# openjamoses/TOSEM-2021-Replication

Hardware: NVIDIA H100
Metric: source MB/s scanned (tokenise + line-hash + classify + aggregate) (higher is better)
Workload: dtype u8

## Files before the change

### tosem-2021-replication_b200/csrc/tsm_api.cu

```cuda
#include <algorithm>
#include <cstdio>
#include <cstdlib>
#include <cstring>
#include <new>
#include <vector>

#include "tsm_device.cuh"

#include "tsm_scan_kernels.cuh"
#include "tsm_scan_walk.cuh"
#include "tsm_reduce_kernels.cuh"
#include "tsm_diff_kernels.cuh"
#include "tsm_blame_kernels.cuh"
#include "tsm_stmt_kernels.cuh"
#include "tsm_lines_kernels.cuh"
#include "tsm_similar_kernels.cuh"

using namespace tsm;

static const char* const kNames[TSM_K] = TSM_CAT_NAMES_INIT;

struct ScratchPool {
  struct Slot { void* p; size_t cap; bool used; };
  std::vector<Slot> slots;
// ... 328 lines not shown
  CU(cudaSetDevice(c->device));
  cudaStream_t st = (cudaStream_t)stream;
  CallOrder order(c, st);
  CU(order.wait());
  rc = upload_index(c, k, st);
  if (rc != TSM_OK) return rc;
  if (c->n_files) CU(cudaMemcpyAsync(c->d_arena, k->arena, (size_t)c->arena_bytes, cudaMemcpyHostToDevice, st));
  c->resident = true;
  c->scanned = false;
  return TSM_OK;
}

static int ensure_event_buffers(tsm_ctx* c, uint32_t flags) {
  if ((flags & TSM_SCAN_ASSERT_EVENTS) && !c->d_aev)
    CU(cudaMalloc((void**)&c->d_aev, sizeof(tsm_assert_event) * (size_t)c->max_events));
  if ((flags & TSM_SCAN_HEADER_EVENTS) && !c->d_hev)
    CU(cudaMalloc((void**)&c->d_hev, sizeof(tsm_header_event) * (size_t)c->max_events));
  return TSM_OK;
}

static ScanParams make_params(const tsm_ctx* c, uint32_t flags) {
  ScanParams p{};
  p.arena = c->d_arena; p.off = c->d_off; p.len = c->d_len; p.ext = c->d_ext; p.grp = c->d_grp;
  p.n_files = c->n_files; p.n_groups = c->n_groups;
  p.unit_file = c->d_unit_file; p.unit_begin = c->d_unit_begin; p.unit_cap = c->unit_cap;
  p.ctrl = c->d_ctrl; p.stats = c->d_stats;
  p.cand = c->d_cand; p.cand_cap = (uint32_t)c->max_events;
  p.hev = c->d_hev; p.hev_cap = (uint32_t)c->max_events;
  p.aev = c->d_aev; p.aev_cap = (uint32_t)c->max_events;
  p.counts = c->d_counts; p.flags = flags; p.four = 4; p.cls_last = 1;
  return p;
}

static int classify_per_sm(tsm_ctx* c, size_t smem) {
  if (c->cls_smem != smem) {
    int per_sm = 0;
    if (cudaOccupancyMaxActiveBlocksPerMultiprocessor(&per_sm, k_classify_t<false>, 256, smem) != cudaSuccess || per_sm < 1) per_sm = 4;
    c->cls_per_sm = per_sm;
    c->cls_smem = smem;
  }
  return c->cls_per_sm;
}

static int launch_scan(tsm_ctx* c, uint32_t flags, cudaStream_t st, const tsm_corpus* host, bool check_files_here = false) {
  int rc = ensure_event_buffers(c, flags);
  if (rc != TSM_OK) return rc;
  ScanParams p = make_params(c, flags);
  const int n = c->n_files;
  c->launches = 0;
  CU(cudaMemsetAsync(c->d_zero, 0, (size_t)(reinterpret_cast<uint8_t*>(c->d_counts) - c->d_zero) +
                     sizeof(unsigned long long) * ((size_t)(c->n_groups + 1) * TSM_K + 4), st));
  if (n) {
    std::vector<int32_t> cut{0};
    if (host) {
      int64_t slab_bytes = 32ll << 20;
      while (c->arena_bytes / slab_bytes + 1 > tsm_ctx::kMaxSlabs) slab_bytes *= 2;
      int64_t next = slab_bytes;
      for (int32_t i = 1; i < n; ++i)
        if ((int64_t)host->off[i] >= next) { cut.push_back(i); next = (int64_t)host->off[i] + slab_bytes; }
      CU(cudaEventRecord(c->ready_ev, st));
      CU(cudaStreamWaitEvent(c->copy_stream, c->ready_ev, 0));
    }
    cut.push_back(n);
    if ((int)cut.size() - 1 > tsm_ctx::kMaxSlabs) return TSM_E_LAYOUT;
    const int es = c->ev_next;
    c->ev_next = (es + 1) % tsm_ctx::kRing;
    fold_events(c, es);
    cudaEvent_t* ev = c->ev[es];
    CU(cudaEventRecord(ev[0], st));
    const int n_slabs = (int)cut.size() - 1;
    const size_t hist = CLS_SMEM_BASE + sizeof(uint32_t) * (c->n_groups <= 16 ? (size_t)c->n_groups * TSM_K : 0);
    const int cls_grid = c->sms * classify_per_sm(c, hist);
    for (int s = 0; s < n_slabs; ++s) {
      const int32_t f0 = cut[(size_t)s], f1 = cut[(size_t)s + 1];
      if (host) {
        if (check_files_here && s == 0) {
          const int rc0 = check_files(host, f0, f1, true, true);
          if (rc0 != TSM_OK) return rc0;
        }
        const size_t b0 = (size_t)host->off[f0], b1 = (size_t)host->off[f1];
        CU(cudaMemcpyAsync(c->d_arena + b0, host->arena + b0, b1 - b0, cudaMemcpyHostToDevice, c->copy_stream));
        CU(cudaEventRecord(c->slab_ev[s], c->copy_stream));
        CU(cudaStreamWaitEvent(st, c->slab_ev[s], 0));
        if (check_files_here && s + 1 < n_slabs) {
          const int rc1 = check_files(host, f1, cut[(size_t)s + 2], true, true);
          if (rc1 != TSM_OK) { cudaStreamSynchronize(c->copy_stream); cudaStreamSynchronize(st); return rc1; }
        }
      }
      p.slab = c->d_slab + s; p.f_begin = f0; p.f_end = f1;
      p.unit_base = (uint32_t)((host ? (int64_t)host->off[f0] : 0) / CH + f0);
      k_plan<<<(f1 - f0 + 255) / 256, 256, 0, st>>>(p);
      CU(cudaGetLastError());
      if (s == 0 && n_slabs == 1) CU(cudaEventRecord(ev[1], st));
      if (flags & TSM_SCAN_REV_B) k_scan_t<true><<<c->sms * SCAN2_CTAS_PER_SM, SCAN2_WARPS * 32, SCAN2_SMEM_B, st>>>(p);
      else k_scan_t<false><<<c->sms * SCAN2_CTAS_PER_SM, SCAN2_WARPS * 32, SCAN2_SMEM, st>>>(p);
      CU(cudaGetLastError());
      if (s + 1 < n_slabs) {
        p.cls_last = 0;
        if (flags & TSM_SCAN_REV_B) k_classify_t<true><<<cls_grid, 256, hist, st>>>(p);
        else k_classify_t<false><<<cls_grid, 256, hist, st>>>(p);
        CU(cudaGetLastError());
        p.cls_last = 1;
      }
    }
    if (n_slabs > 1) CU(cudaEventRecord(ev[1], st));
    CU(cudaEventRecord(ev[2], st));
    if (flags & TSM_SCAN_REV_B) k_classify_t<true><<<cls_grid, 256, hist, st>>>(p);
    else k_classify_t<false><<<cls_grid, 256, hist, st>>>(p);
    CU(cudaGetLastError());
    CU(cudaEventRecord(ev[3], st));
    CU(cudaEventRecord(ev[4], st));
    c->ev_used[es] = (n_slabs == 1);
    c->ev_last = es;
    c->launches = 3 * n_slabs;
    CU(cudaGetLastError());
  }
  c->last_flags = flags;
  c->scanned = true;
  return TSM_OK;
}

extern "C" int tsm_scan_resident(tsm_ctx* c, uint32_t flags, void* stream) {
  if (!c) return TSM_E_ARG;
  flags &= TSM_SCAN_ASSERT_EVENTS | TSM_SCAN_HEADER_EVENTS | TSM_SCAN_REV_B;
  if (!c->resident) return TSM_E_STATE;
  CU(cudaSetDevice(c->device));
  CallOrder order(c, (cudaStream_t)stream);
  CU(order.wait());
  return launch_scan(c, flags, (cudaStream_t)stream, nullptr);
}

extern "C" int tsm_device_counts(tsm_ctx* c, void** dptr, int64_t* n_int64) {
  if (!c || !dptr || !n_int64) return TSM_E_ARG;
  if (!c->scanned) return TSM_E_STATE;
  *dptr = c->d_counts;
  *n_int64 = (int64_t)(c->n_groups + 1) * TSM_K + 4;
  return TSM_OK;
}

extern "C" int tsm_last_launch_count(tsm_ctx* c) { return c ? c->launches : 0; }

#if TSM_PHASE_CLOCKS
extern "C" int tsm_phase_clocks(unsigned long long* out, int n, int reset) {
  if (!out || n < (int)PH_N) return TSM_E_ARG;
  CU(cudaDeviceSynchronize());
  CU(cudaMemcpyFromSymbol(out, g_scan_phase_clk, sizeof(unsigned long long) * PH_N));
  if (reset) {
    const unsigned long long zero[PH_N] = {};
    CU(cudaMemcpyToSymbol(g_scan_phase_clk, zero, sizeof(zero)));
  }
  return TSM_OK;
}
#endif

extern "C" int tsm_last_kernel_ms(tsm_ctx* c, float* ms4) {
  if (!c || !ms4) return TSM_E_ARG;
  if (!c->scanned || c->n_files == 0 || c->ev_last < 0) return TSM_E_STATE;
  CU(cudaSetDevice(c->device));
  cudaEvent_t* ev = c->ev[c->ev_last];
  CU(cudaEventSynchronize(ev[4]));
  for (int i = 0; i < 4; ++i) CU(cudaEventElapsedTime(&ms4[i], ev[i], ev[i + 1]));
  return TSM_OK;
}

extern "C" int tsm_kernel_ms_stats(tsm_ctx* c, double* sum_ms4, int64_t* n_scans, int reset) {
  if (!c) return TSM_E_ARG;
  CU(cudaSetDevice(c->device));
  for (int i = 0; i < tsm_ctx::kRing; ++i) fold_events(c, i);
  if (sum_ms4) for (int k = 0; k < 4; ++k) sum_ms4[k] = c->ms_sum[k];
  if (n_scans) *n_scans = c->ms_n;
  if (reset) { for (double& v : c->ms_sum) v = 0; c->ms_n = 0; }
  return TSM_OK;
}

static int grow_event_buffers(tsm_ctx* c, int64_t need) {
  if (need <= c->max_events) return TSM_OK;
  if (need > 0xFFFFFFF0ll) return TSM_E_CAPACITY;
  unsigned long long* cand = nullptr;
  tsm_assert_event* aev = nullptr;
  tsm_header_event* hev = nullptr;
  const bool ok = cudaMalloc((void**)&cand, sizeof(unsigned long long) * (size_t)need) == cudaSuccess &&
                  (!c->d_aev || cudaMalloc((void**)&aev, sizeof(tsm_assert_event) * (size_t)need) == cudaSuccess) &&
                  (!c->d_hev || cudaMalloc((void**)&hev, sizeof(tsm_header_event) * (size_t)need) == cudaSuccess);
  if (!ok) {
    cudaGetLastError();
    cudaFree(cand); cudaFree(aev); cudaFree(hev);
    return TSM_E_CUDA;
  }
  cudaFree(c->d_cand); cudaFree(c->d_aev); cudaFree(c->d_hev);
  c->d_cand = cand; c->d_aev = aev; c->d_hev = hev;
  c->max_events = need;
  return TSM_OK;
}

static int download_tables(tsm_ctx* c, tsm_result* r, cudaStream_t st) {
  const int n = c->n_files, G = c->n_groups;
  unsigned long long* h_tot = reinterpret_cast<unsigned long long*>(c->h_ctrl + 1);
  CU(cudaMemcpyAsync(c->h_ctrl, c->d_ctrl, sizeof(Ctrl), cudaMemcpyDeviceToHost, st));
  CU(cudaMemcpyAsync(h_tot, c->d_counts + (size_t)(G + 1) * TSM_K, 4 * sizeof(unsigned long long), cudaMemcpyDeviceToHost, st));
  if (r->stats && n) CU(cudaMemcpyAsync(r->stats, c->d_stats, sizeof(tsm_file_stat) * (size_t)n, cudaMemcpyDeviceToHost, st));
  if (r->group_counts) CU(cudaMemcpyAsync(r->group_counts, c->d_counts, sizeof(int64_t) * (size_t)G * TSM_K, cudaMemcpyDeviceToHost, st));
  if (r->global_counts) CU(cudaMemcpyAsync(r->global_counts, c->d_counts + (size_t)G * TSM_K, sizeof(int64_t) * TSM_K, cudaMemcpyDeviceToHost, st));
  CU(cudaStreamSynchronize(st));
  for (int i = 0; i < 4; ++i) r->totals[i] = (int64_t)h_tot[i];
  return TSM_OK;
}

template <typename Event> static void sort_events_by_file(Event* ev, uint32_t m, int32_t n_files) {
  if (m < 2) return;
  std::vector<uint32_t> pos((size_t)n_files + 1, 0);
  for (uint32_t i = 0; i < m; ++i) pos[(size_t)ev[i].file + 1]++;
  for (int32_t f = 0; f < n_files; ++f) pos[(size_t)f + 1] += pos[(size_t)f];
  std::vector<Event> tmp(m);
  std::vector<uint32_t> at(pos.begin(), pos.end() - 1);
  for (uint32_t i = 0; i < m; ++i) tmp[at[ev[i].file]++] = ev[i];
  for (int32_t f = 0; f < n_files; ++f)
    if (pos[(size_t)f + 1] - pos[(size_t)f] > 1)
      std::sort(tmp.begin() + pos[(size_t)f], tmp.begin() + pos[(size_t)f + 1],
                [](const Event& a, const Event& b) { return a.line_off < b.line_off; });
  std::copy(tmp.begin(), tmp.end(), ev);
}

static int download(tsm_ctx* c, tsm_result* r, cudaStream_t st) {
  r->n_aev = 0; r->n_hev = 0;
  int rc = download_tables(c, r, st);
  if (rc != TSM_OK) return rc;
  if (c->h_ctrl->overflow) {
    const Ctrl& k = *c->h_ctrl;
    rc = grow_event_buffers(c, std::max<int64_t>(k.n_cand, std::max(k.n_hev, k.n_aev)));
    if (rc == TSM_OK) rc = launch_scan(c, c->last_flags, st, nullptr);
    if (rc == TSM_OK) rc = download_tables(c, r, st);
    if (rc != TSM_OK) return rc;
    if (c->h_ctrl->overflow) return TSM_E_CAPACITY;
  }
  const bool want_aev = (c->last_flags & TSM_SCAN_ASSERT_EVENTS) && r->aev, want_hev = (c->last_flags & TSM_SCAN_HEADER_EVENTS) && r->hev;
  if ((want_aev && (int64_t)c->h_ctrl->n_aev > r->aev_cap) || (want_hev && (int64_t)c->h_ctrl->n_hev > r->hev_cap)) {
    r->n_aev = c->h_ctrl->n_aev; r->n_hev = c->h_ctrl->n_hev;
    return TSM_E_CAPACITY;
  }
  if (want_aev) {
    const uint32_t m = c->h_ctrl->n_aev;
    CU(cudaMemcpyAsync(r->aev, c->d_aev, sizeof(tsm_assert_event) * (size_t)m, cudaMemcpyDeviceToHost, st));
    CU(cudaStreamSynchronize(st));
    sort_events_by_file(r->aev, m, c->n_files);
    r->n_aev = m;
  } else if (c->last_flags & TSM_SCAN_ASSERT_EVENTS) r->n_aev = c->h_ctrl->n_aev;
  if (want_hev) {
    const uint32_t m = c->h_ctrl->n_hev;
    CU(cudaMemcpyAsync(r->hev, c->d_hev, sizeof(tsm_header_event) * (size_t)m, cudaMemcpyDeviceToHost, st));
    CU(cudaStreamSynchronize(st));
    sort_events_by_file(r->hev, m, c->n_files);
    r->n_hev = m;
  } else if (c->last_flags & TSM_SCAN_HEADER_EVENTS) r->n_hev = c->h_ctrl->n_hev;
  return TSM_OK;
}

extern "C" int tsm_download(tsm_ctx* c, tsm_result* r, void* stream) {
  if (!c || !r) return TSM_E_ARG;
  if (!c->scanned) return TSM_E_STATE;
  CU(cudaSetDevice(c->device));
  CallOrder order(c, (cudaStream_t)stream);
  CU(order.wait());
  return download(c, r, (cudaStream_t)stream);
}

extern "C" int tsm_scan(tsm_ctx* c, const tsm_corpus* k, tsm_result* r, uint32_t flags, void* stream) {
  if (!c || !r) return TSM_E_ARG;
  int rc = check_corpus_head(c, k);
  if (rc != TSM_OK) return rc;
  flags &= TSM_SCAN_ASSERT_EVENTS | TSM_SCAN_HEADER_EVENTS | TSM_SCAN_REV_B;
  CU(cudaSetDevice(c->device));
  cudaStream_t st = (cudaStream_t)stream;
  CallOrder order(c, st);
  CU(order.wait());
  rc = upload_index(c, k, st);
  if (rc != TSM_OK) return rc;
  c->resident = true;
  rc = launch_scan(c, flags, st, k, true);
  if (rc != TSM_OK) { c->resident = false; c->scanned = false; return rc; }
  return download(c, r, st);
}

extern "C" int tsm_reduce(tsm_ctx* c, const uint8_t* flags, const int32_t* repo, const int32_t* case_id,
                          int32_t n_rows, int32_t n_flags, int32_t n_repos, int32_t n_cases,
                          int64_t* out, int64_t* cases_per_repo, void* stream) {
  if (!c || n_rows < 0 || n_flags < 0 || n_repos <= 0 || n_cases <= 0 || !out || (n_rows && (!flags || !repo || !case_id)))
    return TSM_E_ARG;
  for (int32_t i = 0; i < n_rows; ++i)
    if (repo[i] < 0 || repo[i] >= n_repos || case_id[i] < 0 || case_id[i] >= n_cases) return TSM_E_ARG;
  CU(cudaSetDevice(c->device));
  PoolScope pool_scope(&c->pool);
  cudaStream_t st = (cudaStream_t)stream;
  CallOrder order(c, st);
  CU(order.wait());
  const size_t words = ((size_t)n_cases + 31) / 32;
  const size_t nbits = (size_t)(n_flags + 1) * n_repos * words;
  DevBuf b_flags, b_repo, b_case, b_bits, b_out;
  SyncGuard guard(st);
  if (!b_flags.alloc((size_t)n_rows * n_flags) || !b_repo.alloc(sizeof(int32_t) * (size_t)n_rows) ||
      !b_case.alloc(sizeof(int32_t) * (size_t)n_rows) || !b_bits.alloc(sizeof(uint32_t) * nbits) ||
      !b_out.alloc(sizeof(unsigned long long) * (size_t)(n_flags + 1) * n_repos))
    return TSM_E_CUDA;
  uint8_t* d_flags = b_flags.as<uint8_t>(); int32_t *d_repo = b_repo.as<int32_t>(), *d_case = b_case.as<int32_t>();
  uint32_t* d_bits = b_bits.as<uint32_t>();
  unsigned long long* d_out = b_out.as<unsigned long long>();
  int rc = TSM_OK;
// ... 868 lines not shown
```

### tosem-2021-replication_b200/csrc/tsm_scan_kernels.cuh

```cuda
#pragma once
#include "tsm_device.cuh"

namespace tsm {

__constant__ uint32_t c_lut[256];
__constant__ uint32_t c_lut_b[256];
__constant__ uint32_t c_elut[256];
__device__ uint8_t c_cat_slot[TSM_CAT_SLOTS];
__device__ uint16_t c_cat_off[TSM_CAT_NAMED + 1];
__device__ char c_cat_blob[TSM_CAT_BLOB_LEN + 1];

__global__ void k_plan(ScanParams p) {
  const int f = p.f_begin + blockIdx.x * blockDim.x + threadIdx.x;
  const int lane = threadIdx.x & 31;
  if (blockIdx.x == 0 && threadIdx.x == 0) p.ctrl->cls_done = p.ctrl->n_cand;
  uint32_t nu = 0;
  if (f < p.f_end) {
    nu = ((uint32_t)p.len[f] + CH - 1) / CH;
    if (nu != 1) p.stats[f] = tsm_file_stat{0, 0, 0, 0, 0};
  }
  uint32_t incl = nu;
#pragma unroll
  for (int d = 1; d < 32; d <<= 1) {
    uint32_t t = __shfl_up_sync(0xffffffffu, incl, d);
    if (lane >= d) incl += t;
  }
  const uint32_t total = __shfl_sync(0xffffffffu, incl, 31);
  uint32_t base = 0;
  if (lane == 31 && total) base = atomicAdd(&p.slab->n_units, total);
  base = __shfl_sync(0xffffffffu, base, 31);
  uint32_t at = p.unit_base + base + incl - nu;
  for (uint32_t u = 0; u < nu; ++u, ++at) {
    if (at < p.unit_cap) { p.unit_file[at] = (uint32_t)f; p.unit_begin[at] = u * CH; }
    else p.ctrl->overflow = 1;
  }
}

__device__ __forceinline__ uint32_t nl_word(uint32_t w) {
  const uint32_t y = w ^ 0x0A0A0A0Au;
  const uint32_t t = (y & 0x7F7F7F7Fu) + 0x7F7F7F7Fu;
  const uint32_t z = ~(t | y | 0x7F7F7F7Fu);
  return (z * 0x00204081u) >> 28;
}
__device__ __forceinline__ uint32_t spaces_of(unsigned long long w) {
  const unsigned long long x = w ^ 0x2020202020202020ull, k7 = 0x7F7F7F7F7F7F7F7Full;
  const unsigned long long nz = (((x & k7) + k7) | x) & ~k7;
  return nz ? ((uint32_t)__ffsll((long long)nz) - 1u) >> 3 : 8u;
}
struct SmemByte {
  const uint8_t* b;
  __device__ __forceinline__ uint32_t operator()(uint32_t i) const { return b[i]; }
  __device__ __forceinline__ unsigned long long load8(uint32_t i) const {
    const uint32_t a = i & ~7u, sh = 8u * (i & 7u);
    const unsigned long long lo = *reinterpret_cast<const unsigned long long*>(b + a);
    const unsigned long long hi = *reinterpret_cast<const unsigned long long*>(b + a + 8);
    return sh ? (lo >> sh) | (hi << (64u - sh)) : lo;
  }
  __device__ __forceinline__ uint32_t spaces8(uint32_t i) const { return spaces_of(load8(i)); }
};
struct HbmByte {
  const uint8_t* b;
  __device__ __forceinline__ uint32_t operator()(uint32_t i) const { return __ldg(b + i); }
  __device__ __forceinline__ unsigned long long load8(uint32_t i) const {
    const unsigned long long* w = reinterpret_cast<const unsigned long long*>(b) + (i >> 3);
    const uint32_t sh = 8u * (i & 7u);
    const unsigned long long lo = __ldg(w), hi = __ldg(w + 1);
    return sh ? (lo >> sh) | (hi << (64u - sh)) : lo;
  }
  __device__ __forceinline__ uint32_t spaces8(uint32_t i) const { return spaces_of(load8(i)); }
};
struct Accum { uint32_t lines, asserts, hdrs, fixes; unsigned long long digest; };

__device__ __forceinline__ uint32_t warp_reserve(uint32_t* counter, uint32_t n, int lane) {
  uint32_t base = 0;
  if (lane == 0 && n) base = atomicAdd(counter, n);
  return __shfl_sync(0xffffffffu, base, 0);
}

__device__ __forceinline__ const uint32_t* scan_lut() {
  extern __shared__ __align__(128) uint8_t smem[];
  return reinterpret_cast<const uint32_t*>(smem);
}

__device__ __forceinline__ void issue_load(const ScanParams& p, uint8_t* buf, uint64_t* bar, uint32_t fo,
                                           uint32_t size, uint32_t cb) {
  const uint32_t lb = cb ? cb - PRE : 0u;
  const uint32_t le = min(cb + CH + EXT, size);
  const uint32_t bytes = (le - lb + 15u) & ~15u;
  mbar_expect_tx(bar, bytes);
  bulk_load(buf + PRE - (cb - lb), p.arena + (size_t)fo + lb, bytes, bar);
}

struct Unit { uint32_t u, f, cb, fo, size; int ext; };

__device__ __forceinline__ Unit claim_unit(const ScanParams& p, uint32_t n_units, int lane) {
  Unit x{0, 0, 0, 0, 0, 0};
  if (lane == 0) x.u = atomicAdd(&p.slab->work, 1u);
  x.u = __shfl_sync(0xffffffffu, x.u, 0);
  if (x.u < n_units) {
    x.f = p.unit_file[p.unit_base + x.u];
    x.cb = p.unit_begin[p.unit_base + x.u];
    x.fo = (uint32_t)p.off[x.f];
    x.size = (uint32_t)p.len[x.f];
    x.ext = p.ext[x.f];
  }
  return x;
}

constexpr uint32_t CC_W = 1, CC_IDENT = 2, CC_STOP = 4;
constexpr uint32_t CLS_CAT_OFF_N = (TSM_CAT_NAMED + 2) & ~1u;
constexpr uint32_t CLS_CAT_WORDS = ((TSM_CAT_SLOTS + 2 * CLS_CAT_OFF_N + TSM_CAT_BLOB_LEN + 15) / 16) * 4;
constexpr uint32_t CLS_SMEM_BASE = 4 * (512 + CLS_CAT_WORDS + 4 * 1024 + 4);
constexpr uint32_t E_FIRST = (1u << 0) | (1u << 5) | (1u << 9) | (1u << 17) | (1u << 21) | (1u << 23) | (1u << 25) |
                             (1u << 27) | (1u << 29) | (1u << 30);

struct FileBytes {
  const unsigned long long* base; uint32_t cur_blk; unsigned long long w;
  uint32_t blk0; unsigned long long w0, w1, w2, w3;
  __device__ __forceinline__ FileBytes(const uint8_t* b, uint32_t first_byte)
      : base(reinterpret_cast<const unsigned long long*>(b)), cur_blk(0xFFFFFFFFu), w(0), blk0(first_byte >> 3) {
    w0 = __ldg(base + blk0); w1 = __ldg(base + blk0 + 1); w2 = __ldg(base + blk0 + 2); w3 = __ldg(base + blk0 + 3);
  }
  __device__ __forceinline__ unsigned long long word(uint32_t blk) const {
    const uint32_t d = blk - blk0;
    if (d < 4u) return d < 2u ? (d == 0u ? w0 : w1) : (d == 2u ? w2 : w3);
    return __ldg(base + blk);
  }
  __device__ __forceinline__ uint32_t get(uint32_t i) {
    const uint32_t blk = i >> 3;
    if (blk != cur_blk) { w = word(blk); cur_blk = blk; }
    return (uint32_t)(w >> (8u * (i & 7u))) & 0xFFu;
  }
  __device__ __forceinline__ unsigned long long get8(uint32_t i) const {
    const uint32_t blk = i >> 3, sh = 8u * (i & 7u);
    const unsigned long long lo = word(blk);
    if (sh == 0) return lo;
    return (lo >> sh) | (word(blk + 1) << (64u - sh));
  }
};

__device__ __forceinline__ unsigned long long low_bytes(unsigned long long v, uint32_t n) {
  return n >= 8 ? v : (v & ((1ull << (8u * n)) - 1ull));
}

__device__ __forceinline__ int stem_lookup(FileBytes& rd, uint32_t s, uint32_t n) {
  if (n < 2 || n > 9) return 0;
  const unsigned long long v = low_bytes(rd.get8(s), n);
  const uint32_t c9 = n == 9 ? rd.get(s + 8) : 0u;
  switch (n) {
    case 2:
      if (v == 0x5145ull) return 1;
      if (v == 0x454Eull) return 2;
      if (v == 0x5447ull) return 5;
      if (v == 0x4547ull) return 6;
      if (v == 0x544Cull) return 7;
      if (v == 0x454Cull) return 8;
      return 0;
    case 4:
      if (v == 0x45555254ull) return 3;
      if (v == 0x5241454Eull) return 9;
      return 0;
    case 5:
      if (v == 0x45534C4146ull) return 4;
      if (v == 0x574F524854ull) return 12;
      return 0;
    case 8: return v == 0x51455F54414F4C46ull ? 10 : 0;
    case 9: return (v == 0x455F454C42554F44ull && c9 == 'Q') ? 11 : 0;
    default: return 0;
  }
}

__device__ __forceinline__ int bare_assert_category(FileBytes& rd, uint32_t e0, uint32_t en, const uint32_t* elut, int deflt = 3,
                                                    bool not_prefix = true) {
  if (not_prefix && en >= 4 && (uint32_t)rd.get8(e0) == 0x20746F6Eu) return 2;
  uint32_t D = 0, A = 0;
  for (uint32_t a = 0; a < en; a += 8) {
    unsigned long long w = rd.get8(e0 + a);
    if (en - a < 8) w &= (1ull << (8u * (en - a))) - 1ull;
    const uint32_t lo = (uint32_t)w, hi = (uint32_t)(w >> 32);
#pragma unroll
    for (int k = 0; k < 4; ++k) { D = ((D + D) | E_FIRST) & elut[__byte_perm(lo, 0, 0x4440 + k)]; A |= D; }
#pragma unroll
    for (int k = 0; k < 4; ++k) { D = ((D + D) | E_FIRST) & elut[__byte_perm(hi, 0, 0x4440 + k)]; A |= D; }
  }
  if (((A & (1u << 4)) && (A & (1u << 8))) || (A & (1u << 16))) return 4;
  if (A & (1u << 20)) return 3;
  if (A & (1u << 22)) return 1;
  if (A & (1u << 24)) return 2;
  if (A & (1u << 26)) return 8;
  if (A & (1u << 28)) return 6;
  if (A & (1u << 29)) return 7;
  if (A & (1u << 30)) return 5;
  return deflt;
}

__device__ __noinline__ bool ident_eq(FileBytes& rd, uint32_t s, uint32_t n, const char* name, uint32_t len) {
  if (n != len) return false;
  for (uint32_t k = 0; k < len; ++k)
    if (rd.get(s + k) != (uint8_t)name[k]) return false;
  return true;
}

constexpr uint32_t BQ_CAP = 1024;

#ifndef TSM_CLS_MINB
#define TSM_CLS_MINB 1
#endif
template <bool REVB>
__global__ void __launch_bounds__(256, TSM_CLS_MINB) k_classify_t(ScanParams p) {
  extern __shared__ __align__(16) uint32_t csm[];
  uint32_t* cls = csm;
  uint32_t* elut = csm + 256;
  uint8_t* cat_slot = reinterpret_cast<uint8_t*>(csm + 512);
  uint16_t* cat_off = reinterpret_cast<uint16_t*>(cat_slot + TSM_CAT_SLOTS);
  uint8_t* cat_blob = reinterpret_cast<uint8_t*>(cat_off + CLS_CAT_OFF_N);
  uint4* bq = reinterpret_cast<uint4*>(csm + 512 + CLS_CAT_WORDS);
  uint32_t* bqn = csm + 512 + CLS_CAT_WORDS + 4 * BQ_CAP;
  uint32_t* hist = bqn + 4;
  const bool use_smem = p.n_groups <= 16;
  for (int i = threadIdx.x; i < 256; i += blockDim.x) {
    const uint32_t c = (uint32_t)i;
    cls[i] = (is_w(c) ? CC_W : 0u) | (is_ident(c) ? CC_IDENT : 0u) | ((c == '(' || c == '\n') ? CC_STOP : 0u);
    elut[i] = c_elut[i];
  }
  for (int i = threadIdx.x; i < TSM_CAT_SLOTS; i += blockDim.x) cat_slot[i] = c_cat_slot[i];
  for (int i = threadIdx.x; i < TSM_CAT_NAMED + 1; i += blockDim.x) cat_off[i] = c_cat_off[i];
  for (int i = threadIdx.x; i < TSM_CAT_BLOB_LEN; i += blockDim.x) cat_blob[i] = (uint8_t)c_cat_blob[i];
  if (use_smem) for (int i = threadIdx.x; i < p.n_groups * TSM_K; i += blockDim.x) hist[i] = 0;
  if (threadIdx.x == 0) *bqn = 0;
  __syncthreads();
  auto count = [&](uint32_t f, int cat) {
    const uint32_t g = p.grp ? p.grp[f] : 0u;
    if (use_smem) atomicAdd(&hist[g * TSM_K + cat], 1u);
    else {
      atomicAdd(&p.counts[(size_t)g * TSM_K + cat], 1ull);
      atomicAdd(&p.counts[(size_t)p.n_groups * TSM_K + cat], 1ull);
    }
  };
  const uint32_t n = min(p.ctrl->n_cand, p.cand_cap), n0 = min(p.ctrl->cls_done, n);
  const bool want_ev = (p.flags & TSM_SCAN_ASSERT_EVENTS) != 0;
  constexpr bool revb = REVB;
  for (uint32_t i = n0 + blockIdx.x * blockDim.x + threadIdx.x; i < n; i += gridDim.x * blockDim.x) {
    const unsigned long long cd = p.cand[i];
    const uint32_t f = (uint32_t)(cd >> 32), line_off = (uint32_t)cd;
    const uint32_t size = (uint32_t)p.len[f];
    FileBytes rd(p.arena + (size_t)(uint32_t)p.off[f], line_off);
    uint32_t q = line_off;
    while (q < size && (cls[rd.get(q)] & CC_W)) ++q;
    const uint32_t t0 = q;
    uint32_t stop = size;
    for (uint32_t wb = t0 & ~7u; wb < size; wb += 8) {
      unsigned long long w = rd.word(wb >> 3);
      const unsigned long long x1 = w ^ 0x2828282828282828ull, x2 = w ^ 0x0A0A0A0A0A0A0A0Aull;
      const unsigned long long k7 = 0x7F7F7F7F7F7F7F7Full;
      unsigned long long z = (~(((x1 & k7) + k7) | x1 | k7)) | (~(((x2 & k7) + k7) | x2 | k7));
      if (wb < t0) z &= ~0ull << (8u * (t0 - wb));
      if (z) { stop = wb + ((uint32_t)__ffsll((long long)z) - 1u) / 8u; break; }
    }
    stop = min(stop, size);
    uint32_t last = stop;
    while (last > t0 && (cls[rd.get(last - 1)] & CC_W)) --last;
    uint32_t Ls = last;
    while (Ls > t0 && (cls[rd.get(Ls - 1)] & CC_IDENT)) --Ls;
    uint32_t tlen = last - t0;
    const uint32_t tlen_a = tlen, Ln = last - Ls;
    int cat = 0;
    bool done = false;
    uint32_t def_e0 = 0, def_en = 0;
    if (revb) {
      const bool macro = ident_eq(rd, Ls, Ln, "BOOST_CHECK", 11) || ident_eq(rd, Ls, Ln, "NTA_CHECK", 9);
      const bool bare6 = tlen == 6 && low_bytes(rd.get8(t0), 6) == 0x747265737361ull;
      const bool full = macro || p.ext[f] == TSM_EXT_JAVA;
      uint32_t fe = last;
      if (full || ((macro || bare6) && stop < size && rd.get(stop) == '(')) {
        uint32_t le = stop;
        while (le < size && rd.get(le) != '\n') ++le;
        fe = le;
        while (fe > t0 && (cls[rd.get(fe - 1)] & CC_W)) --fe;
      }
      if (ident_eq(rd, Ls, Ln, "BOOST_CHECK_EQUAL", 17)) { cat = 1; done = true; }
      else if ((macro || bare6) && stop < size && rd.get(stop) == '(') {
        uint32_t x = stop + 1;
        while (x < fe && (cls[rd.get(x)] & CC_W)) ++x;
        if (x < fe && rd.get(x) == '!' && !(x + 1 < fe && rd.get(x + 1) == '=')) cat = 4;
        else cat = bare_assert_category(rd, x, fe > x ? fe - x : 0u, elut, macro ? 0 : 3, false);
        done = true;
      }
      if (full) tlen = fe - t0;
    }
    if (Ln >= 7) {
      const unsigned long long h7 = low_bytes(rd.get8(Ls), 7);
      if (h7 == 0x5F544345505845ull || h7 == 0x5F545245535341ull) { cat = stem_lookup(rd, Ls + 7, Ln - 7); done = true; }
    }
    if (!done && tlen_a >= 6) {
      const unsigned long long h = rd.get8(t0);
      const bool a6 = low_bytes(h, 6) == 0x747265737361ull;
      if (a6 && tlen_a == 6) { cat = 3; done = true; }
      else if (a6 && tlen_a >= 8 && ((h >> 48) & 0xFF) == 0x20) {
        done = true;
        def_e0 = t0 + 7; def_en = tlen_a - 7;
      }
    }
    if (!done && Ln >= 6) {
      const unsigned long long h = rd.get8(Ls);
      if (low_bytes(h, 6) == 0x747265737361ull) {
        if (Ln == 7 && ((h >> 48) & 0xFF) == '_') cat = 3;
        else {
          cat = TSM_CAT_OTHER;
          uint32_t hh = 0x811C9DC5u;
          for (uint32_t j = 0; j < Ln; j += 8) {
            unsigned long long w = rd.get8(Ls + j);
            const uint32_t nb = min(8u, Ln - j);
#pragma unroll
            for (uint32_t k = 0; k < 8; ++k) {
              if (k < nb) hh = (hh ^ ((uint32_t)w & 0xFFu)) * 0x01000193u;
              w >>= 8;
            }
          }
          const int id = cat_slot[(hh * TSM_CAT_HASH_MULT) >> 23];
          if (id && (uint32_t)(cat_off[id + 1] - cat_off[id]) == Ln) {
            const uint8_t* name = cat_blob + cat_off[id];
            bool ok = true;
            for (uint32_t j = 0; j < Ln; j += 8) {
              unsigned long long w = rd.get8(Ls + j);
              const uint32_t nb = min(8u, Ln - j);
              for (uint32_t k = 0; k < nb; ++k) { ok &= ((uint32_t)w & 0xFFu) == (uint32_t)name[j + k]; w >>= 8; }
            }
            if (ok) cat = id;
          }
        }
      }
    }
    uint32_t ev_slot = 0xFFFFFFFFu;
    if (want_ev) {
      unsigned long long hacc = 0; uint32_t hr = 0;
      for (uint32_t j = 0; j < tlen; ++j) {
        hacc = fold61(hacc + rotl61((unsigned long long)rd.get(t0 + j), hr));
        hr += 8; if (hr >= 61) hr -= 61;
      }
      const uint32_t slot = atomicAdd(&p.ctrl->n_aev, 1u);
      if (slot < p.aev_cap) {
        tsm_assert_event ev;
        ev.file = f; ev.line_off = line_off; ev.stmt_off = t0;
        ev.stmt_len = (uint16_t)min(tlen, 65535u); ev.cat = (uint16_t)cat;
        ev.ident_off = Ls; ev.ident_len = (uint16_t)min(Ln, 65535u); ev.pad = 0;
        ev.stmt_hash = mix_hash(canon61(hacc), tlen);
        p.aev[slot] = ev;
        ev_slot = slot;
      } else p.ctrl->overflow = 1;
    }
    if (def_en) {
      const uint32_t slot = atomicAdd(bqn, 1u);
      if (slot < BQ_CAP) { bq[slot] = make_uint4(f, def_e0, def_en, ev_slot); continue; }
      cat = bare_assert_category(rd, def_e0, def_en, elut);
      if (ev_slot != 0xFFFFFFFFu) p.aev[ev_slot].cat = (uint16_t)cat;
    }
    count(f, cat);
  }
  __syncthreads();
  {
    const uint32_t nq = min(*bqn, BQ_CAP);
    for (uint32_t t = threadIdx.x; t < nq; t += blockDim.x) {
      const uint4 e = bq[t];
      FileBytes rd(p.arena + (size_t)(uint32_t)p.off[e.x], e.y);
      const int cat = bare_assert_category(rd, e.y, e.z, elut);
      if (e.w != 0xFFFFFFFFu) p.aev[e.w].cat = (uint16_t)cat;
      count(e.x, cat);
    }
  }
  if (p.cls_last) {
    unsigned long long t0 = 0, t1 = 0, t2 = 0, t3 = 0;
    for (int f = blockIdx.x * blockDim.x + threadIdx.x; f < p.n_files; f += gridDim.x * blockDim.x) {
      const tsm_file_stat s = p.stats[f];
      t0 += s.n_lines; t1 += s.n_assert; t2 += s.n_headers; t3 += s.n_fixture;
    }
#pragma unroll
    for (int d = 16; d; d >>= 1) {
      t0 += __shfl_xor_sync(0xffffffffu, t0, d); t1 += __shfl_xor_sync(0xffffffffu, t1, d);
      t2 += __shfl_xor_sync(0xffffffffu, t2, d); t3 += __shfl_xor_sync(0xffffffffu, t3, d);
    }
    if ((threadIdx.x & 31) == 0) {
      unsigned long long* tot = p.counts + (size_t)(p.n_groups + 1) * TSM_K;
      if (t0) atomicAdd(&tot[0], t0);
      if (t1) atomicAdd(&tot[1], t1);
      if (t2) atomicAdd(&tot[2], t2);
      if (t3) atomicAdd(&tot[3], t3);
    }
  }
  if (use_smem) {
    __syncthreads();
    for (int i = threadIdx.x; i < p.n_groups * TSM_K; i += blockDim.x) {
      const uint32_t v = hist[i];
      if (v) {
        atomicAdd(&p.counts[i], (unsigned long long)v);
        atomicAdd(&p.counts[(size_t)p.n_groups * TSM_K + (i & (TSM_K - 1))], (unsigned long long)v);
      }
    }
  }
}

template __global__ void k_classify_t<false>(ScanParams);
template __global__ void k_classify_t<true>(ScanParams);

}
```

Baseline: 615,700.

## Stage candidate line windows in shared memory and compute statement bounds with SWAR masks

The classify kernel now has each warp cooperatively load a 64-byte window per candidate into a shared-memory stash with coalesced loads. It also prefetches the next candidate index. Statement bounds (first non-blank, stop char, trailing ident) are found with SWAR byte masks over the window instead of byte-by-byte loops. Smaller changes: category tables are copied as words, name comparison uses 8-byte XOR, min blocks per SM goes from 1 to 5, and group totals are flushed with fewer atomics. Optional phase-clock instrumentation is added behind a macro. The cost is more shared memory per block and extra register pressure, and the larger minimum-blocks bound could force register spills.

```diff
diff --git a/tosem-2021-replication_b200/csrc/tsm_api.cu b/tosem-2021-replication_b200/csrc/tsm_api.cu
--- a/tosem-2021-replication_b200/csrc/tsm_api.cu
+++ b/tosem-2021-replication_b200/csrc/tsm_api.cu
@@ -504,6 +504,18 @@
   return TSM_OK;
 }
 #endif
+#if TSM_CLS_PHASE_CLOCKS
+extern "C" int tsm_cls_phase_clocks(unsigned long long* out, int n, int reset) {
+  if (!out || n < (int)CP_N) return TSM_E_ARG;
+  CU(cudaDeviceSynchronize());
+  CU(cudaMemcpyFromSymbol(out, g_cls_phase_clk, sizeof(unsigned long long) * CP_N));
+  if (reset) {
+    const unsigned long long zero[CP_N] = {};
+    CU(cudaMemcpyToSymbol(g_cls_phase_clk, zero, sizeof(zero)));
+  }
+  return TSM_OK;
+}
+#endif
 
 extern "C" int tsm_last_kernel_ms(tsm_ctx* c, float* ms4) {
   if (!c || !ms4) return TSM_E_ARG;
diff --git a/tosem-2021-replication_b200/csrc/tsm_scan_kernels.cuh b/tosem-2021-replication_b200/csrc/tsm_scan_kernels.cuh
--- a/tosem-2021-replication_b200/csrc/tsm_scan_kernels.cuh
+++ b/tosem-2021-replication_b200/csrc/tsm_scan_kernels.cuh
@@ -6,9 +6,9 @@
 __constant__ uint32_t c_lut[256];
 __constant__ uint32_t c_lut_b[256];
 __constant__ uint32_t c_elut[256];
-__device__ uint8_t c_cat_slot[TSM_CAT_SLOTS];
-__device__ uint16_t c_cat_off[TSM_CAT_NAMED + 1];
-__device__ char c_cat_blob[TSM_CAT_BLOB_LEN + 1];
+__device__ __align__(16) uint8_t c_cat_slot[TSM_CAT_SLOTS];
+__device__ __align__(16) uint16_t c_cat_off[(TSM_CAT_NAMED + 2) & ~1u];
+__device__ __align__(16) char c_cat_blob[(TSM_CAT_BLOB_LEN + 4) & ~3u];
 
 __global__ void k_plan(ScanParams p) {
   const int f = p.f_begin + blockIdx.x * blockDim.x + threadIdx.x;
@@ -110,15 +110,19 @@
 constexpr uint32_t CC_W = 1, CC_IDENT = 2, CC_STOP = 4;
 constexpr uint32_t CLS_CAT_OFF_N = (TSM_CAT_NAMED + 2) & ~1u;
 constexpr uint32_t CLS_CAT_WORDS = ((TSM_CAT_SLOTS + 2 * CLS_CAT_OFF_N + TSM_CAT_BLOB_LEN + 15) / 16) * 4;
-constexpr uint32_t CLS_SMEM_BASE = 4 * (512 + CLS_CAT_WORDS + 4 * 1024 + 4);
+constexpr uint32_t CLS_WARPS = 8;
+constexpr uint32_t CLS_WIN_WORDS = 8;
+constexpr uint32_t CLS_SLOT_WORDS = CLS_WIN_WORDS + 1;
+constexpr uint32_t CLS_STASH_WORDS = CLS_WARPS * 32 * CLS_SLOT_WORDS;
+constexpr uint32_t CLS_SMEM_BASE = 4 * (512 + CLS_CAT_WORDS + 4 * 1024 + 4) + 8 * CLS_STASH_WORDS;
 constexpr uint32_t E_FIRST = (1u << 0) | (1u << 5) | (1u << 9) | (1u << 17) | (1u << 21) | (1u << 23) | (1u << 25) |
                              (1u << 27) | (1u << 29) | (1u << 30);
 
-struct FileBytes {
-  const unsigned long long* base; uint32_t cur_blk; unsigned long long w;
+struct HbmWords {
+  const unsigned long long* base;
   uint32_t blk0; unsigned long long w0, w1, w2, w3;
-  __device__ __forceinline__ FileBytes(const uint8_t* b, uint32_t first_byte)
-      : base(reinterpret_cast<const unsigned long long*>(b)), cur_blk(0xFFFFFFFFu), w(0), blk0(first_byte >> 3) {
+  __device__ __forceinline__ HbmWords(const uint8_t* b, uint32_t first_byte)
+      : base(reinterpret_cast<const unsigned long long*>(b)), blk0(first_byte >> 3) {
     w0 = __ldg(base + blk0); w1 = __ldg(base + blk0 + 1); w2 = __ldg(base + blk0 + 2); w3 = __ldg(base + blk0 + 3);
   }
   __device__ __forceinline__ unsigned long long word(uint32_t blk) const {
@@ -126,24 +130,124 @@
     if (d < 4u) return d < 2u ? (d == 0u ? w0 : w1) : (d == 2u ? w2 : w3);
     return __ldg(base + blk);
   }
+};
+struct StagedWords {
+  const unsigned long long* base;
+  const unsigned long long* win;
+  uint32_t blk0;
+  __device__ __forceinline__ unsigned long long word(uint32_t blk) const {
+    const uint32_t d = blk - blk0;
+    return d < CLS_WIN_WORDS ? win[d] : __ldg(base + blk);
+  }
+};
+
+template <class Words>
+struct ByteReader : Words {
+  uint32_t cur_blk = 0xFFFFFFFFu; unsigned long long w = 0;
+  __device__ __forceinline__ explicit ByteReader(const Words& src) : Words(src) {}
   __device__ __forceinline__ uint32_t get(uint32_t i) {
     const uint32_t blk = i >> 3;
-    if (blk != cur_blk) { w = word(blk); cur_blk = blk; }
+    if (blk != cur_blk) { w = this->word(blk); cur_blk = blk; }
     return (uint32_t)(w >> (8u * (i & 7u))) & 0xFFu;
   }
   __device__ __forceinline__ unsigned long long get8(uint32_t i) const {
     const uint32_t blk = i >> 3, sh = 8u * (i & 7u);
-    const unsigned long long lo = word(blk);
+    const unsigned long long lo = this->word(blk);
     if (sh == 0) return lo;
-    return (lo >> sh) | (word(blk + 1) << (64u - sh));
+    return (lo >> sh) | (this->word(blk + 1) << (64u - sh));
   }
 };
+using FileBytes = ByteReader<HbmWords>;
+using WinBytes = ByteReader<StagedWords>;
+
+__device__ __forceinline__ uint32_t eq_bytes(uint32_t w, uint32_t r) {
+  const uint32_t y = w ^ r;
+  return ~(((y & 0x7F7F7F7Fu) + 0x7F7F7F7Fu) | y | 0x7F7F7F7Fu);
+}
+__device__ __forceinline__ uint32_t range_bytes(uint32_t w, uint32_t rl, uint32_t rh) {
+  const uint32_t x = w & 0x7F7F7F7Fu;
+  return (x + rl) & ~(x + rh) & ~w & 0x80808080u;
+}
+__device__ __forceinline__ uint32_t flags4(uint32_t z) { return (z * 0x00204081u) >> 28; }
+struct WinMasks { unsigned long long blank, stop, ident; };
+__device__ __forceinline__ WinMasks window_masks(const unsigned long long (&w)[CLS_WIN_WORDS]) {
+  WinMasks m{0, 0, 0};
+#pragma unroll
+  for (int k = 0; k < 2 * (int)CLS_WIN_WORDS; ++k) {
+    const uint32_t v = (uint32_t)(w[k >> 1] >> (32 * (k & 1)));
+    const uint32_t lf = eq_bytes(v, 0x0A0A0A0Au);
+    const uint32_t bl = eq_bytes(v, 0x20202020u) | (range_bytes(v, 0x77777777u, 0x72727272u) & ~lf);
+    const uint32_t st = eq_bytes(v, 0x28282828u) | lf;
+    const uint32_t id = range_bytes(v | 0x20202020u, 0x1F1F1F1Fu, 0x05050505u) |
+                        range_bytes(v, 0x50505050u, 0x46464646u) | eq_bytes(v, 0x5F5F5F5Fu);
+    m.blank |= (unsigned long long)flags4(bl) << (4 * k);
+    m.stop |= (unsigned long long)flags4(st) << (4 * k);
+    m.ident |= (unsigned long long)flags4(id) << (4 * k);
+  }
+  return m;
+}
+struct StmtBounds { uint32_t t0, stop, last, Ls; };
+__device__ __forceinline__ StmtBounds statement_bounds(const unsigned long long* win, const unsigned long long* file,
+                                                       uint32_t line_off, uint32_t size) {
+  uint32_t ws = line_off & ~7u;
+  unsigned long long from = ~0ull << (line_off - ws);
+  uint32_t t0 = 0xFFFFFFFFu, stop, lnb = 0, Ls = 0, run = 0;
+  unsigned long long w[CLS_WIN_WORDS];
+#pragma unroll
+  for (uint32_t k = 0; k < CLS_WIN_WORDS; ++k) w[k] = win[k];
+  for (;;) {
+    WinMasks m = window_masks(w);
+    const int lim = (int)size - (int)ws;
+    const unsigned long long beyond = lim <= 0 ? ~0ull : (lim >= 64 ? 0ull : ~0ull << lim);
+    m.blank &= ~beyond; m.ident &= ~beyond; m.stop |= beyond;
+    if (t0 == 0xFFFFFFFFu) {
+      const unsigned long long nb = ~m.blank & from;
+      if (nb) {
+        t0 = ws + (uint32_t)__ffsll((long long)nb) - 1u;
+        from = ~0ull << (t0 - ws);
+        run = t0;
+      }
+    }
+    if (t0 != 0xFFFFFFFFu) {
+      const unsigned long long st = m.stop & from;
+      const unsigned long long reg = st ? ((st & (0ull - st)) - 1ull) & from : from;
+      const unsigned long long nbr = ~m.blank & reg, id = m.ident & reg;
+      if (nbr) {
+        const uint32_t hb = 63u - (uint32_t)__clzll((long long)nbr);
+        lnb = ws + hb + 1u;
+        if (!((id >> hb) & 1ull)) Ls = lnb;
+        else {
+          const unsigned long long gaps = ~id & ((2ull << hb) - 1ull);
+          Ls = gaps ? ws + 64u - (uint32_t)__clzll((long long)gaps) : run;
+        }
+      }
+      if (st) { stop = ws + (uint32_t)__ffsll((long long)st) - 1u; break; }
+      if (id >> 63) { if (~id) run = ws + 64u - (uint32_t)__clzll((long long)~id); }
+      else run = ws + 64u;
+    }
+    ws += 64u; from = ~0ull;
+#pragma unroll
+    for (uint32_t k = 0; k < CLS_WIN_WORDS; ++k) w[k] = __ldg(file + (ws >> 3) + k);
+  }
+  StmtBounds b;
+  b.t0 = t0;
+  b.stop = min(stop, size);
+  b.last = lnb ? lnb : b.stop;
+  b.Ls = lnb ? Ls : b.last;
+  return b;
+}
 
 __device__ __forceinline__ unsigned long long low_bytes(unsigned long long v, uint32_t n) {
   return n >= 8 ? v : (v & ((1ull << (8u * n)) - 1ull));
 }
-
-__device__ __forceinline__ int stem_lookup(FileBytes& rd, uint32_t s, uint32_t n) {
+__device__ __forceinline__ unsigned long long smem_bytes8(const uint8_t* b, uint32_t o) {
+  const uint32_t* w = reinterpret_cast<const uint32_t*>(b) + (o >> 2);
+  const uint32_t sh = 8u * (o & 3u), w0 = w[0], w1 = w[1], w2 = w[2];
+  return (unsigned long long)__funnelshift_r(w0, w1, sh) | ((unsigned long long)__funnelshift_r(w1, w2, sh) << 32);
+}
+
+template <class R>
+__device__ __forceinline__ int stem_lookup(R& rd, uint32_t s, uint32_t n) {
   if (n < 2 || n > 9) return 0;
   const unsigned long long v = low_bytes(rd.get8(s), n);
   const uint32_t c9 = n == 9 ? rd.get(s + 8) : 0u;
@@ -170,7 +274,8 @@
   }
 }
 
-__device__ __forceinline__ int bare_assert_category(FileBytes& rd, uint32_t e0, uint32_t en, const uint32_t* elut, int deflt = 3,
+template <class R>
+__device__ __forceinline__ int bare_assert_category(R& rd, uint32_t e0, uint32_t en, const uint32_t* elut, int deflt = 3,
                                                     bool not_prefix = true) {
   if (not_prefix && en >= 4 && (uint32_t)rd.get8(e0) == 0x20746F6Eu) return 2;
   uint32_t D = 0, A = 0;
@@ -194,7 +299,8 @@
   return deflt;
 }
 
-__device__ __noinline__ bool ident_eq(FileBytes& rd, uint32_t s, uint32_t n, const char* name, uint32_t len) {
+template <class R>
+__device__ __noinline__ bool ident_eq(R& rd, uint32_t s, uint32_t n, const char* name, uint32_t len) {
   if (n != len) return false;
   for (uint32_t k = 0; k < len; ++k)
     if (rd.get(s + k) != (uint8_t)name[k]) return false;
@@ -203,12 +309,41 @@
 
 constexpr uint32_t BQ_CAP = 1024;
 
+#ifndef TSM_CLS_PHASE_CLOCKS
+#define TSM_CLS_PHASE_CLOCKS 0
+#endif
+enum ClsPhase { CP_SETUP, CP_LOAD, CP_BOUNDS, CP_RULES, CP_EVENT, CP_DEFER, CP_TOTALS, CP_FLUSH, CP_N };
+#if TSM_CLS_PHASE_CLOCKS
+__device__ unsigned long long g_cls_phase_clk[CP_N];
+#endif
+struct ClsClock {
+#if TSM_CLS_PHASE_CLOCKS
+  unsigned long long acc[CP_N], sink;
+  long long t;
+  __device__ __forceinline__ ClsClock() : acc{}, sink(0) { t = clock64(); }
+  __device__ __forceinline__ void mark(int ph, unsigned long long wait_for = 0) {
+    asm volatile("xor.b64 %0, %0, %1;" : "+l"(sink) : "l"(wait_for));
+    const long long now = clock64();
+    acc[ph] += (unsigned long long)(now - t);
+    t = now;
+  }
+  __device__ __forceinline__ void flush() {
+    if ((threadIdx.x & 31) == 0)
+      for (int k = 0; k < CP_N; ++k) atomicAdd(&g_cls_phase_clk[k], acc[k] + (sink & 0ull));
+  }
+#else
+  __device__ __forceinline__ void mark(int, unsigned long long = 0) {}
+  __device__ __forceinline__ void flush() {}
+#endif
+};
+
 #ifndef TSM_CLS_MINB
-#define TSM_CLS_MINB 1
+#define TSM_CLS_MINB 5
 #endif
 template <bool REVB>
 __global__ void __launch_bounds__(256, TSM_CLS_MINB) k_classify_t(ScanParams p) {
   extern __shared__ __align__(16) uint32_t csm[];
+  ClsClock clk;
   uint32_t* cls = csm;
   uint32_t* elut = csm + 256;
   uint8_t* cat_slot = reinterpret_cast<uint8_t*>(csm + 512);
@@ -216,21 +351,29 @@
   uint8_t* cat_blob = reinterpret_cast<uint8_t*>(cat_off + CLS_CAT_OFF_N);
   uint4* bq = reinterpret_cast<uint4*>(csm + 512 + CLS_CAT_WORDS);
   uint32_t* bqn = csm + 512 + CLS_CAT_WORDS + 4 * BQ_CAP;
-  uint32_t* hist = bqn + 4;
+  unsigned long long* stash = reinterpret_cast<unsigned long long*>(bqn + 4);
+  uint32_t* hist = reinterpret_cast<uint32_t*>(stash + CLS_STASH_WORDS);
   const bool use_smem = p.n_groups <= 16;
   for (int i = threadIdx.x; i < 256; i += blockDim.x) {
     const uint32_t c = (uint32_t)i;
-    cls[i] = (is_w(c) ? CC_W : 0u) | (is_ident(c) ? CC_IDENT : 0u) | ((c == '(' || c == '\n') ? CC_STOP : 0u);
+    if (REVB) cls[i] = (is_w(c) ? CC_W : 0u) | (is_ident(c) ? CC_IDENT : 0u) | ((c == '(' || c == '\n') ? CC_STOP : 0u);
     elut[i] = c_elut[i];
   }
-  for (int i = threadIdx.x; i < TSM_CAT_SLOTS; i += blockDim.x) cat_slot[i] = c_cat_slot[i];
-  for (int i = threadIdx.x; i < TSM_CAT_NAMED + 1; i += blockDim.x) cat_off[i] = c_cat_off[i];
-  for (int i = threadIdx.x; i < TSM_CAT_BLOB_LEN; i += blockDim.x) cat_blob[i] = (uint8_t)c_cat_blob[i];
+  {
+    static_assert(TSM_CAT_SLOTS % 4 == 0 && CLS_CAT_OFF_N % 2 == 0 && 4 * CLS_CAT_WORDS >= TSM_CAT_SLOTS + 2 * CLS_CAT_OFF_N +
+                  sizeof(c_cat_blob) + 11 && sizeof(c_cat_off) == 2 * CLS_CAT_OFF_N && sizeof(c_cat_blob) % 4 == 0, "category table words");
+    constexpr int n_slot = TSM_CAT_SLOTS / 4, n_off = CLS_CAT_OFF_N / 2, n_blob = (int)sizeof(c_cat_blob) / 4;
+    for (int i = threadIdx.x; i < n_slot + n_off + n_blob; i += blockDim.x) {
+      if (i < n_slot) reinterpret_cast<uint32_t*>(cat_slot)[i] = reinterpret_cast<const uint32_t*>(c_cat_slot)[i];
+      else if (i < n_slot + n_off) reinterpret_cast<uint32_t*>(cat_off)[i - n_slot] = reinterpret_cast<const uint32_t*>(c_cat_off)[i - n_slot];
+      else reinterpret_cast<uint32_t*>(cat_blob)[i - n_slot - n_off] = reinterpret_cast<const uint32_t*>(c_cat_blob)[i - n_slot - n_off];
+    }
+  }
   if (use_smem) for (int i = threadIdx.x; i < p.n_groups * TSM_K; i += blockDim.x) hist[i] = 0;
   if (threadIdx.x == 0) *bqn = 0;
   __syncthreads();
-  auto count = [&](uint32_t f, int cat) {
-    const uint32_t g = p.grp ? p.grp[f] : 0u;
+  auto group_of = [&](uint32_t f) { return p.grp ? (uint32_t)p.grp[f] : 0u; };
+  auto count = [&](uint32_t g, int cat) {
     if (use_smem) atomicAdd(&hist[g * TSM_K + cat], 1u);
     else {
       atomicAdd(&p.counts[(size_t)g * TSM_K + cat], 1ull);
@@ -240,30 +383,39 @@
   const uint32_t n = min(p.ctrl->n_cand, p.cand_cap), n0 = min(p.ctrl->cls_done, n);
   const bool want_ev = (p.flags & TSM_SCAN_ASSERT_EVENTS) != 0;
   constexpr bool revb = REVB;
-  for (uint32_t i = n0 + blockIdx.x * blockDim.x + threadIdx.x; i < n; i += gridDim.x * blockDim.x) {
-    const unsigned long long cd = p.cand[i];
+  const uint32_t lane = threadIdx.x & 31u;
+  unsigned long long* slots = stash + (threadIdx.x >> 5) * 32u * CLS_SLOT_WORDS;
+  const unsigned long long* win = slots + lane * CLS_SLOT_WORDS;
+  const uint32_t wb0 = n0 + blockIdx.x * blockDim.x + (threadIdx.x & ~31u), stride = gridDim.x * blockDim.x;
+  unsigned long long cd_next = wb0 + lane < n ? p.cand[wb0 + lane] : 0ull;
+  clk.mark(CP_SETUP, n0);
+  for (uint32_t wb = wb0; wb < n; wb += stride) {
+    const uint32_t i = wb + lane;
+    const unsigned long long cd = cd_next;
+    cd_next = i + stride < n ? p.cand[i + stride] : 0ull;
     const uint32_t f = (uint32_t)(cd >> 32), line_off = (uint32_t)cd;
-    const uint32_t size = (uint32_t)p.len[f];
-    FileBytes rd(p.arena + (size_t)(uint32_t)p.off[f], line_off);
-    uint32_t q = line_off;
-    while (q < size && (cls[rd.get(q)] & CC_W)) ++q;
-    const uint32_t t0 = q;
-    uint32_t stop = size;
-    for (uint32_t wb = t0 & ~7u; wb < size; wb += 8) {
-      unsigned long long w = rd.word(wb >> 3);
-      const unsigned long long x1 = w ^ 0x2828282828282828ull, x2 = w ^ 0x0A0A0A0A0A0A0A0Aull;
-      const unsigned long long k7 = 0x7F7F7F7F7F7F7F7Full;
-      unsigned long long z = (~(((x1 & k7) + k7) | x1 | k7)) | (~(((x2 & k7) + k7) | x2 | k7));
-      if (wb < t0) z &= ~0ull << (8u * (t0 - wb));
-      if (z) { stop = wb + ((uint32_t)__ffsll((long long)z) - 1u) / 8u; break; }
-    }
-    stop = min(stop, size);
-    uint32_t last = stop;
-    while (last > t0 && (cls[rd.get(last - 1)] & CC_W)) --last;
-    uint32_t Ls = last;
-    while (Ls > t0 && (cls[rd.get(Ls - 1)] & CC_IDENT)) --Ls;
+    const uint32_t size = (uint32_t)p.len[f], g = group_of(f);
+    const unsigned long long* file = reinterpret_cast<const unsigned long long*>(p.arena + (size_t)(uint32_t)p.off[f]);
+    const unsigned long long* src = file + (line_off >> 3);
+    unsigned long long v[8];
+#pragma unroll
+    for (uint32_t r = 0; r < 8; ++r) {
+      const auto* s = reinterpret_cast<const unsigned long long*>(
+          __shfl_sync(0xffffffffu, reinterpret_cast<unsigned long long>(src), 4u * r + (lane >> 3)));
+      v[r] = __ldg(s + (lane & 7u));
+    }
+    __syncwarp();
+#pragma unroll
+    for (uint32_t r = 0; r < 8; ++r) slots[(4u * r + (lane >> 3)) * CLS_SLOT_WORDS + (lane & 7u)] = v[r];
+    __syncwarp();
+    clk.mark(CP_LOAD, size ^ g);
+    if (i >= n) continue;
+    const StmtBounds bd = statement_bounds(win, file, line_off, size);
+    const uint32_t t0 = bd.t0, stop = bd.stop, last = bd.last, Ls = bd.Ls;
+    WinBytes rd(StagedWords{file, win, line_off >> 3});
     uint32_t tlen = last - t0;
     const uint32_t tlen_a = tlen, Ln = last - Ls;
+    clk.mark(CP_BOUNDS, Ls);
     int cat = 0;
     bool done = false;
     uint32_t def_e0 = 0, def_en = 0;
@@ -319,18 +471,16 @@
           }
           const int id = cat_slot[(hh * TSM_CAT_HASH_MULT) >> 23];
           if (id && (uint32_t)(cat_off[id + 1] - cat_off[id]) == Ln) {
-            const uint8_t* name = cat_blob + cat_off[id];
+            const uint32_t name = cat_off[id];
             bool ok = true;
-            for (uint32_t j = 0; j < Ln; j += 8) {
-              unsigned long long w = rd.get8(Ls + j);
-              const uint32_t nb = min(8u, Ln - j);
-              for (uint32_t k = 0; k < nb; ++k) { ok &= ((uint32_t)w & 0xFFu) == (uint32_t)name[j + k]; w >>= 8; }
-            }
+            for (uint32_t j = 0; j < Ln; j += 8)
+              ok &= low_bytes(rd.get8(Ls + j) ^ smem_bytes8(cat_blob, name + j), min(8u, Ln - j)) == 0ull;
             if (ok) cat = id;
           }
         }
       }
     }
+    clk.mark(CP_RULES, (uint32_t)cat);
     uint32_t ev_slot = 0xFFFFFFFFu;
     if (want_ev) {
       unsigned long long hacc = 0; uint32_t hr = 0;
@@ -349,25 +499,28 @@
         ev_slot = slot;
       } else p.ctrl->overflow = 1;
     }
+    clk.mark(CP_EVENT, ev_slot);
     if (def_en) {
       const uint32_t slot = atomicAdd(bqn, 1u);
-      if (slot < BQ_CAP) { bq[slot] = make_uint4(f, def_e0, def_en, ev_slot); continue; }
+      if (slot < BQ_CAP) { bq[slot] = make_uint4(f, def_e0, def_en, ev_slot); clk.mark(CP_RULES); continue; }
       cat = bare_assert_category(rd, def_e0, def_en, elut);
       if (ev_slot != 0xFFFFFFFFu) p.aev[ev_slot].cat = (uint16_t)cat;
     }
-    count(f, cat);
+    count(g, cat);
+    clk.mark(CP_RULES);
   }
   __syncthreads();
   {
     const uint32_t nq = min(*bqn, BQ_CAP);
     for (uint32_t t = threadIdx.x; t < nq; t += blockDim.x) {
       const uint4 e = bq[t];
-      FileBytes rd(p.arena + (size_t)(uint32_t)p.off[e.x], e.y);
+      FileBytes rd(HbmWords(p.arena + (size_t)(uint32_t)p.off[e.x], e.y));
       const int cat = bare_assert_category(rd, e.y, e.z, elut);
       if (e.w != 0xFFFFFFFFu) p.aev[e.w].cat = (uint16_t)cat;
-      count(e.x, cat);
-    }
-  }
+      count(group_of(e.x), cat);
+    }
+  }
+  clk.mark(CP_DEFER);
   if (p.cls_last) {
     unsigned long long t0 = 0, t1 = 0, t2 = 0, t3 = 0;
     for (int f = blockIdx.x * blockDim.x + threadIdx.x; f < p.n_files; f += gridDim.x * blockDim.x) {
@@ -387,16 +540,21 @@
       if (t3) atomicAdd(&tot[3], t3);
     }
   }
+  clk.mark(CP_TOTALS);
   if (use_smem) {
     __syncthreads();
     for (int i = threadIdx.x; i < p.n_groups * TSM_K; i += blockDim.x) {
       const uint32_t v = hist[i];
-      if (v) {
-        atomicAdd(&p.counts[i], (unsigned long long)v);
-        atomicAdd(&p.counts[(size_t)p.n_groups * TSM_K + (i & (TSM_K - 1))], (unsigned long long)v);
-      }
-    }
-  }
+      if (v) atomicAdd(&p.counts[i], (unsigned long long)v);
+    }
+    for (int k = threadIdx.x; k < TSM_K; k += blockDim.x) {
+      uint32_t v = 0;
+      for (int gi = 0; gi < p.n_groups; ++gi) v += hist[gi * TSM_K + k];
+      if (v) atomicAdd(&p.counts[(size_t)p.n_groups * TSM_K + k], (unsigned long long)v);
+    }
+  }
+  clk.mark(CP_FLUSH);
+  clk.flush();
 }
 
 template __global__ void k_classify_t<false>(ScanParams);
```

Result: faster. 625,400, median of 6 (+1.6%).
